# jasperlinthorst/reveal

Measured on AMD Instinct MI355X. Metric: Mbp/s indexed+MUM-anchored (reveal rem), higher is better.
Workload: dtype int32

## Files before the change

### reveal_amd/csrc/rv_cascade.hip

```cpp
#include "rv_index.h"
#include "rv_cascade.h"
#include "rv_leaf.h"
#include <algorithm>
#include <string.h>
#include <stdio.h>
#include <stdlib.h>
#include <chrono>

namespace {

constexpr int TB = 256;
constexpr u32 NONE = 0xFFFFFFFFu;
#ifdef RV_SA64
constexpr int KEY_SHIFT = 40;
#else
constexpr int KEY_SHIFT = 32;
#endif
constexpr u64 KEY_LOW = (1ull << KEY_SHIFT) - 1;

struct CasIv { sa_t a0, a1, b0, b1; };
struct CasRes { sa_t qa, qb; u32 ql, lead, trail, state; };
enum { C_NCHILD = 0, C_NUND = 1, C_NWIT = 2, C_ERR = 3, C_MAXN = 4, C_LO = 5, C_HI = 6, C_LEVELS = 7, C_NSOLVED = 8, C_NUNSOLVED = 9, C_NRETRY = 10, C_TICKET = 11,
       C_NANCH = 12  };

// ... 14 lines not shown
__device__ inline u64 shfl_up64(u64 v, int d) {
    const u32 lo = __shfl_up((u32)v, d, 64), hi = __shfl_up((u32)(v >> 32), d, 64);
    return ((u64)hi << 32) | lo;
}
__device__ inline void seg_atomic_max64(u64 *__restrict__ dst, u32 child, u64 val, bool active) {
    const int lane = threadIdx.x & 63;
    if (!active) { child = NONE; val = 0; }
    val = rv_wave_seg_max_u64(child, val);
    const u32 nc = __shfl_down(child, 1, 64);
    const bool last = lane == 63 || nc != child;
    if (active && last && val > dst[child]) atomicMax((unsigned long long *)&dst[child], (unsigned long long)val);
}
__device__ inline void seg_atomic_max32(u32 *__restrict__ dst, u32 child, u32 val, bool active) {
    const int lane = threadIdx.x & 63;
    if (!active) { child = NONE; val = 0; }
    val = rv_wave_seg_max_u32(child, val);
    const u32 nc = __shfl_down(child, 1, 64);
    const bool last = lane == 63 || nc != child;
    if (active && last && val > dst[child]) atomicMax(&dst[child], val);
}

constexpr int WT_ITEMS = 8;
constexpr int WT_TILE = TB * WT_ITEMS;
constexpr int WT_REGIONS = 64;
__global__ __launch_bounds__(TB) void k_cas_witness(const sa_t *__restrict__ SA, const lcp_t *__restrict__ LCP, const uint8_t *__restrict__ BWT, int64_t n,
                                                    u32 minl, sa_t *__restrict__ w_pos, u32 *__restrict__ w_val, u32 *__restrict__ w_rank, u32 cap , u32 *__restrict__ counters ) {
    __shared__ __attribute__((aligned(16))) u32 sl0[WT_TILE + 8];
    __shared__ __attribute__((aligned(16))) uint8_t ss0[WT_TILE + 32];
    u32 *const sl = sl0 + 3;
    uint8_t *const ss = ss0 + 15;
    const int64_t j0 = (int64_t)blockIdx.x * WT_TILE;
    if (j0 + WT_TILE + 2 <= n && sizeof(lcp_t) == 4) {
        const uint4 *L4 = reinterpret_cast<const uint4 *>(LCP + j0);
        uint4 *d4 = reinterpret_cast<uint4 *>(sl + 1);
        for (int k = threadIdx.x; k < WT_TILE / 4; k += TB) d4[k] = L4[k];
        const uint4 *B4 = reinterpret_cast<const uint4 *>(BWT + j0);
        for (int k = threadIdx.x; k < WT_TILE / 16; k += TB) {
            uint4 v = B4[k];
            v.x = (v.x >> 7) & 0x01010101u; v.y = (v.y >> 7) & 0x01010101u; v.z = (v.z >> 7) & 0x01010101u; v.w = (v.w >> 7) & 0x01010101u;
            reinterpret_cast<uint4 *>(ss + 1)[k] = v;
        }
        if (threadIdx.x == 0) { sl[0] = j0 > 0 ? (u32)LCP[j0 - 1] : 0u; ss[0] = j0 > 0 ? (uint8_t)(BWT[j0 - 1] >> 7) : (uint8_t)0; }
        if (threadIdx.x == 1) { sl[WT_TILE + 1] = (u32)LCP[j0 + WT_TILE]; ss[WT_TILE + 1] = (uint8_t)(BWT[j0 + WT_TILE] >> 7); }
        if (threadIdx.x == 2) sl[WT_TILE + 2] = (u32)LCP[j0 + WT_TILE + 1];
    } else {
        for (int k = threadIdx.x; k < WT_TILE + 3; k += TB) { const int64_t j = j0 - 1 + k; sl[k] = (j >= 0 && j < n) ? (u32)LCP[j] : 0u; }
        for (int k = threadIdx.x; k < WT_TILE + 2; k += TB) { const int64_t j = j0 - 1 + k; ss[k] = (j >= 0 && j < n) ? (uint8_t)(BWT[j] >> 7) : (uint8_t)0; }
// ... 773 lines not shown
    std::sort(CA.begin(), CA.end(), [](const RvIntv &x, const RvIntv &y) { return x.begin < y.begin; });
    std::sort(CB.begin(), CB.end(), [](const RvIntv &x, const RvIntv &y) { return x.begin < y.begin; });
    if (CA.empty() || CB.empty()) GIVE_UP("an empty sample");
    const bool chain = CA.size() > 1 || CB.size() > 1;
    if (chain && ws.opt.no_cascade_chain) GIVE_UP("several sequences per sample (switched off)");
    if (n >= ((int64_t)1 << 32) - 2) GIVE_UP("index above 2^32 positions");
#ifdef RV_SA64
    if ((u64)h->maxlcp >= (1ull << 24) || n >= ((int64_t)1 << 40)) GIVE_UP("bid word too narrow");
#endif
    CasIv root; root.a0 = root.a1 = root.b0 = root.b1 = 0;
    root.a0 = (sa_t)CA[0].begin; root.a1 = (sa_t)CA[0].end; root.b0 = (sa_t)CB[0].begin; root.b1 = (sa_t)CB[0].end;
    if (root.a0 >= root.a1 || root.b0 >= root.b1 || (int64_t)root.a1 > h->nsep[0] || (int64_t)root.b0 <= h->nsep[0]) GIVE_UP("an empty sample");

    const sa_t *SA = h->dSA.as<sa_t>(); const lcp_t *LCP = h->dLCP.as<lcp_t>(); const uint8_t *BWT = h->dBWT.as<uint8_t>();

    const int64_t ntile = ceil_div(n, RV_PAIR_TILE);
    DBuf &bcnt = ws.misc[14], &btab = ws.misc[2], &bslot = ws.misc[3], &bovf = ws.misc[4], &bout = ws.misc[5];
    if (bcnt.cap == 0) { RV_TRY(bcnt.reserve(64)); RV_HIP(hipMemsetAsync(bcnt.p, 0, 64, q)); }
    RV_TRY(btab.reserve((size_t)(ntile + 1) * 3 * sizeof(u32)));
    RV_TRY(bslot.reserve((size_t)ntile * RV_PAIR_SLOTS * sizeof(RvPairRec)));
    if (bovf.cap < 4096 * sizeof(RvPairRec)) RV_TRY(bovf.reserve(4096 * sizeof(RvPairRec)));
    if (bout.cap < 4096 * sizeof(RvPairRec)) RV_TRY(bout.reserve(sizeof(RvPairRec) * (size_t)std::max<int64_t>(4096, n / 64)));
    u32 *tilecnt = btab.as<u32>(), *tileovf = tilecnt + (ntile + 1), *tileoff = tileovf + (ntile + 1);
    u32 M = reuse ? cb.M : 0;
    for (int attempt = 0; !reuse; attempt++) {
        if (attempt == 3) { rv_set_error("cascade: scan buffer sizing failed"); return -1; }
        const size_t ocap = bout.cap / sizeof(RvPairRec) - RV_PAIR_HDR, vcap = bovf.cap / sizeof(RvPairRec);
        hipEvent_t ev_a, ev_b;
        (void)h->prof.attach(RV_K_SCAN_PAIR, (double)n * 8.0, &ev_a, &ev_b);
        RV_TRY(rv_scan_pair_launch(ws, SA, LCP, n, BWT, (sa_t)h->nsep[0], (int)minl, bslot.as<RvPairRec>(), bovf.as<RvPairRec>(),
                                   (u32)std::min<size_t>(vcap, 0xffffffffu), bcnt.as<u32>(), tilecnt, tileovf, nullptr, nullptr, 0, ev_a, ev_b));
        RV_TRY(rv_exclusive_sum_u32(ws, tilecnt, tileoff, ntile + 1));
        RV_TRY(rv_pair_compact_launch(ws, bslot.as<RvPairRec>(), bovf.as<RvPairRec>(), tilecnt, tileovf, tileoff, ntile, bout.as<RvPairRec>(),
                                      (u32)std::min<size_t>(ocap, 0xffffffffu), bcnt.as<u32>(), nullptr, (u32)std::min<size_t>(vcap, 0xffffffffu)));
        u32 hdr[4];
        RV_TRY(rv_read_back(ws, hdr, bout.p, sizeof hdr));
        const u32 total = hdr[0], novf = hdr[1];
        if (total <= ocap && novf <= vcap) { M = total; break; }
        if (novf > vcap) RV_TRY(bovf.reserve((size_t)novf * sizeof(RvPairRec)));
        if (total > ocap) RV_TRY(bout.reserve(((size_t)total + RV_PAIR_HDR) * sizeof(RvPairRec)));
    }
    if (verbose) tp[1] = cas_now();
    out->cands = M;
    struct ProfSpan { Workspace &w; int id; ~ProfSpan() { w.prof_end(id); } } span{ws, ws.prof_begin(RV_K_CASCADE, 5.0 * (double)n)};
    if (M == 0) GIVE_UP("no match at the top level");
    const RvPairRec *recs = bout.as<RvPairRec>() + RV_PAIR_HDR;
    cb.M = M;

    const int64_t rcap64 = std::min<int64_t>(n / WT_REGIONS + WT_TILE, std::max<int64_t>(16384, n / 1024));
    const u32 wcap = (u32)std::min<int64_t>(rcap64 * WT_REGIONS, 0x7fffffff);
    const int64_t ccap64 = n / (int64_t)minl + 16;
    if (ccap64 >= 0x7fffffff) GIVE_UP("too many sub-indices possible");
    const u32 ccap = (u32)ccap64;
    DBuf &k0 = cb.d[0], &k1 = cb.d[1], &v0 = cb.d[2], &v1 = cb.d[3], &bpa = cb.d[4], &bpb = cb.d[5], &blen = cb.d[6], &bcc = cb.d[7], &bwp = cb.d[8], &bwv = cb.d[9],
         &bwc = cb.d[10], &biv = cb.d[11], &bbest = cb.d[12], &bwm = cb.d[13], &bdep = cb.d[14], &bres = cb.d[15], &bctr = cb.d[16], &bund = cb.d[17], &bsz = cb.d[18];
    RV_TRY(k0.reserve((size_t)M * 8)); RV_TRY(k1.reserve((size_t)M * 8)); RV_TRY(v0.reserve((size_t)M * 4)); RV_TRY(v1.reserve((size_t)M * 4));
    RV_TRY(bpa.reserve((size_t)M * sizeof(sa_t))); RV_TRY(bpb.reserve((size_t)M * sizeof(sa_t))); RV_TRY(blen.reserve((size_t)M * 4)); RV_TRY(bcc.reserve((size_t)M * 4));
    RV_TRY(bwp.reserve((size_t)wcap * sizeof(sa_t))); RV_TRY(bwv.reserve((size_t)wcap * 4)); RV_TRY(bwc.reserve((size_t)wcap * 4));
    RV_TRY(biv.reserve((size_t)ccap * sizeof(CasIv))); RV_TRY(bbest.reserve((size_t)ccap * 8)); RV_TRY(bwm.reserve((size_t)ccap * 4)); RV_TRY(bdep.reserve((size_t)ccap * 4));
    RV_TRY(bres.reserve((size_t)ccap * sizeof(CasRes))); RV_TRY(bctr.reserve(64)); RV_TRY(bund.reserve((size_t)ccap * 4));
    u32 *counters = bctr.as<u32>();
    RV_HIP(hipMemsetAsync(counters, 0, 64, q));

    DBuf &bwp0 = cb.d[19], &bwv0 = cb.d[20], &bwr = cb.d[21], &bwrk = cb.d[22], &bwrk0 = cb.d[23];
    RV_TRY(bwp0.reserve((size_t)wcap * sizeof(sa_t))); RV_TRY(bwv0.reserve((size_t)wcap * 4)); RV_TRY(bwr.reserve(2 * WT_REGIONS * 4 + 64));
    RV_TRY(bwrk.reserve((size_t)wcap * 4)); RV_TRY(bwrk0.reserve((size_t)wcap * 4));
    u32 hc[16];
    u32 NW = reuse ? cb.NW : 0;
    if (!reuse) {
        u32 *wreg = bwr.as<u32>();
        RV_HIP(hipMemsetAsync(wreg, 0, 2 * WT_REGIONS * 4, q));
        const u32 wrcap = wcap / WT_REGIONS;
        hipLaunchKernelGGL(k_cas_witness, dim3((unsigned)ceil_div(n, WT_TILE)), dim3(TB), 0, q, SA, LCP, BWT, n, minl, bwp0.as<sa_t>(), bwv0.as<u32>(), bwrk0.as<u32>(), wrcap, wreg);
        RV_LAUNCH_CHECK();
        {
            const unsigned mb = (unsigned)ceil_div((int64_t)M, TB);
            hipLaunchKernelGGL(k_cas_keys, dim3(mb), dim3(TB), 0, q, recs, M, k0.as<u64>(), v0.as<u32>());
            RV_LAUNCH_CHECK();
            int in1 = 0;
            RV_TRY(rv_radix_sort_pairs<u32>(ws, k0.as<u64>(), v0.as<u32>(), k1.as<u64>(), v1.as<u32>(), (int64_t)M, 0, bitlen64((u64)n), &in1));
            hipLaunchKernelGGL(k_cas_gather, dim3(mb), dim3(TB), 0, q, recs, (const u32 *)(in1 ? v1.as<u32>() : v0.as<u32>()), M, bpa.as<sa_t>(), bpb.as<sa_t>(),
                               blen.as<u32>(), bcc.as<u32>());
            RV_LAUNCH_CHECK();
        }
        u32 hreg[2 * WT_REGIONS];
        RV_TRY(rv_read_back(ws, hreg, wreg, WT_REGIONS * 4));
        u32 wmaxc = 0;
        for (int r = 0; r < WT_REGIONS; r++) { hreg[WT_REGIONS + r] = NW; NW += hreg[r]; wmaxc = std::max(wmaxc, hreg[r]); }
        out->witnesses = NW;
        if (wmaxc > wrcap) GIVE_UP("too many repeat witnesses (a repetitive input)");
        if (NW) {
            RV_HIP(hipMemcpyAsync(wreg + WT_REGIONS, hreg + WT_REGIONS, WT_REGIONS * 4, hipMemcpyHostToDevice, q));
            RV_HIP(hipStreamSynchronize(q));
            hipLaunchKernelGGL(k_cas_wpack, dim3((unsigned)std::max<int64_t>(1, ceil_div((int64_t)wmaxc, TB)), WT_REGIONS), dim3(TB), 0, q, (const sa_t *)bwp0.as<sa_t>(),
                               (const u32 *)bwv0.as<u32>(), (const u32 *)bwrk0.as<u32>(), wrcap, (const u32 *)wreg, (const u32 *)(wreg + WT_REGIONS), bwp.as<sa_t>(), bwv.as<u32>(),
                               bwrk.as<u32>());
            RV_LAUNCH_CHECK();
        }
        cb.NW = NW;
        if (chain) {
            const char *why = nullptr;
            RV_TRY(cas_lineage(h, cb, M, NW, minl, CA, CB, &why));
            if (why) { cb.lin_picks = 0; cb.lin_rest.clear(); GIVE_UP(why); }
        }
    } else {
        if (chain && cb.lin_picks == 0) GIVE_UP("the chain of rest sub-indices was not decided");
        RV_HIP(hipMemsetAsync(bcc.p, 0, (size_t)M * 4, q));
        out->witnesses = NW;
    }
    const sa_t *wp = bwp.as<sa_t>(); const u32 *wv = bwv.as<u32>();
    CasDanger dg; memset(&dg, 0, sizeof dg);
    u32 dwalk_nmed = 0; const u32 *dwalk_boff = nullptr, *dwalk_mlist = nullptr;
    if (danger) {
        if (NW) {
            RV_TRY(k0.reserve((size_t)NW * 8)); RV_TRY(k1.reserve((size_t)NW * 8)); RV_TRY(v0.reserve((size_t)NW * 4)); RV_TRY(v1.reserve((size_t)NW * 4));
            const unsigned wb = (unsigned)ceil_div((int64_t)NW, TB);
            hipLaunchKernelGGL(k_cas_wkeys, dim3(wb), dim3(TB), 0, q, (const u32 *)bwrk.as<u32>(), NW, k0.as<u64>(), v0.as<u32>());
            RV_LAUNCH_CHECK();
            int in1 = 0;
            RV_TRY(rv_radix_sort_pairs<u32>(ws, k0.as<u64>(), v0.as<u32>(), k1.as<u64>(), v1.as<u32>(), (int64_t)NW, 0, bitlen64((u64)n), &in1));
// ... 207 lines not shown
```

### reveal_amd/csrc/rv_common.h

```cpp
#pragma once
#include <mutex>
#include <thread>
#include <vector>
#include <utility>
#include <hip/hip_runtime.h>
#include <stdint.h>
#include <string.h>
#include <stddef.h>
#include <vector>
#include <string>

#ifdef RV_SA64
typedef int64_t  sa_t;
typedef uint32_t lcp_t;
#else
typedef int32_t  sa_t;
typedef int32_t  lcp_t;
#endif

typedef unsigned long long u64;
typedef unsigned int       u32;

void rv_set_error(const char *fmt, ...);

// ... 51 lines not shown
    X(no_text_jump, "RV_NO_TEXT_JUMP", 0) \
    X(far_table, "RV_FAR_TABLE", 0) \
    X(no_slow_class, "RV_NO_SLOW_CLASS", 0) \
    X(no_dwalk_blocks, "RV_NO_DWALK_BLOCKS", 0) \
    X(no_pub_twins, "RV_NO_PUB_TWINS", 0) \
    X(sa_no_text, "RV_SA_NO_TEXT", 0) \
    X(text_mode, "RV_TEXT_MODE", -1) \
    X(carry_ch, "RV_CARRY_CH", -1) \
    X(rs_bits, "RV_RS_BITS", 8) \
    X(rs_xcd, "RV_RS_XCD", 1) \
    X(rs_cnt16, "RV_RS_CNT16", 1) \
    X(rs_no_digit_bytes, "RV_RS_NO_DIGIT_BYTES", 0) \
    X(diag_table, "RV_DIAG_TABLE", -1) \
    X(no_cascade_chain, "RV_NO_CASCADE_CHAIN", 0) \
    X(casm_rank_count, "RV_CASM_RANK_COUNT", 0) \
    X(casm_big_min, "RV_CASM_BIG_MIN", -1) \
    X(casm_no_big, "RV_CASM_NO_BIG", 0) \
    X(casm_big_root, "RV_CASM_BIG_ROOT", 1 << 22) \
    X(casm_big_total, "RV_CASM_BIG_TOTAL", 1 << 26) \
    X(lock_any, "RV_LOCK_ANY", 0) \
    X(presel_dev_min, "RV_PRESEL_DEV_MIN", 65536) \
    X(scan_v1, "RV_SCAN_V1", 0) \
    X(pick_threads, "RV_PICK_THREADS", 0) \
    X(cascade_prio, "RV_CASCADE_PRIO", 0)
struct RvOptions {
#define RV_X_(f, name, def) int64_t f = def;
    RV_OPTION_LIST(RV_X_)
#undef RV_X_
    int64_t *find(const char *name) {
#define RV_X_(f, nm, def) if (strcmp(name, nm) == 0) return &f;
        RV_OPTION_LIST(RV_X_)
#undef RV_X_
        return nullptr;
    }
};
extern int g_rv_launch_trace;
static inline bool rv_launch_trace_on() { return g_rv_launch_trace != 0; }
#define RV_LAUNCH_CHECK()                                                                      \
    do {                                                                                       \
        RV_HIP(hipGetLastError());                                                             \
        if (rv_launch_trace_on()) {                                                            \
            fprintf(stderr, "launch %s:%d\n", __FILE__, __LINE__);                             \
            fflush(stderr);                                                                    \
            RV_HIP(hipDeviceSynchronize());                                                    \
        }                                                                                      \
    } while (0)

// ... 191 lines not shown
        for (auto &b : sa) b.release();
    }
};

std::mutex &rv_trim_mutex();
struct SaScratchInUse {
    Workspace &w; bool was;
    SaScratchInUse(Workspace &x) : w(x) { std::lock_guard<std::mutex> g(rv_trim_mutex()); was = w.sa_in_use; w.sa_in_use = true; }
    ~SaScratchInUse() { std::lock_guard<std::mutex> g(rv_trim_mutex()); w.sa_in_use = was; }
};

int rv_exclusive_sum_u32(Workspace &ws, const u32 *in, u32 *out, int64_t n);
int rv_exclusive_sum_u64(Workspace &ws, const u64 *in, u64 *out, int64_t n);
int rv_inclusive_max_u32(Workspace &ws, const u32 *in, u32 *out, int64_t n);
int rv_inclusive_max_u64(Workspace &ws, const u64 *in, u64 *out, int64_t n);

int rv_radix_passes(const Workspace &ws, int nbits);
template <class V>
int rv_radix_sort_pairs(Workspace &ws, u64 *k0, V *v0, u64 *k1, V *v1, int64_t n,
                        int bit_lo, int bit_hi, int *result_in_1, bool first_digits = false);
uint8_t *rv_radix_first_digits(Workspace &ws, int64_t n, int bit_lo, int bit_hi);

int rv_read_back(Workspace &ws, void *dst, const void *dsrc, size_t bytes);

int rv_h2d_copy(Workspace &ws, const void *pinned_src, void *dst, size_t bytes);

struct RvSaStats {
    int    sigma, bits, k0;
    int    rounds;
    int64_t sorted_elems;
    int    radix_passes;
    int    diag_table;
    int64_t far_pairs;
    int64_t lcp_list;
};
int rv_build_sa(Workspace &ws, const uint8_t *T, int64_t n, sa_t *SA, RvSaStats *st,
                lcp_t *LCP = nullptr, uint8_t *BWT = nullptr, sa_t side_sep = 0, u32 *d_maxlcp = nullptr, bool *fused_done = nullptr,
                const int64_t *seps = nullptr, int nseps = 0);
int rv_build_inverse(Workspace &ws, const sa_t *SA, sa_t *SAi, int64_t n);
int rv_build_inverse_checked(Workspace &ws, const sa_t *SA, sa_t *SAi, int64_t n);
int rv_build_lcp(Workspace &ws, const uint8_t *T, const sa_t *SA, bool by_rank, lcp_t *LCP, int64_t n, u32 *d_maxlcp, uint8_t *BWT, sa_t side_sep);
int rv_build_bwt(Workspace &ws, const uint8_t *T, const sa_t *SA, int64_t n, uint8_t *BWT, sa_t side_sep);
```

### reveal_amd/csrc/rv_prims.hip

```cpp
#include "rv_common.h"
#include <string.h>

namespace {

constexpr int SCAN_THREADS = 256;
constexpr int SCAN_ITEMS   = 8;
constexpr int SCAN_TILE    = SCAN_THREADS * SCAN_ITEMS;

template <class T> struct OpSum {
    __device__ static T id() { return (T)0; }
    __device__ static T f(T a, T b) { return a + b; }
};
template <class T> struct OpMax {
    __device__ static T id() { return (T)0; }
    __device__ static T f(T a, T b) { return a > b ? a : b; }
};

template <class T> __device__ inline T shfl_up_t(T v, int d) { return __shfl_up(v, d, 64); }
template <> __device__ inline u64 shfl_up_t<u64>(u64 v, int d) {
    u32 lo = __shfl_up((u32)v, d, 64), hi = __shfl_up((u32)(v >> 32), d, 64);
    return ((u64)hi << 32) | lo;
}

template <class T, class Op>
// ... 336 lines not shown
        have_digits = dn != nullptr;
        u64 *tk = ki; ki = ko; ko = tk;
        V *tv = vi; vi = vo; vo = tv;
        flip ^= 1;
    }
    *result_in_1 = flip;
    return 0;
}

__global__ __launch_bounds__(256) void k_h2d_copy(const uint4 *__restrict__ src, uint4 *__restrict__ dst, size_t n16) {
    for (size_t i = (size_t)blockIdx.x * 256 + threadIdx.x; i < n16; i += (size_t)gridDim.x * 256) dst[i] = src[i];
}
int rv_read_back(Workspace &ws, void *dst, const void *dsrc, size_t bytes) {
    RV_TRY(ws.hpin.reserve(bytes < 4096 ? 4096 : bytes));
    if (!ws.ev_rb) RV_HIP(hipEventCreateWithFlags(&ws.ev_rb, hipEventDisableTiming));
    RV_HIP(hipMemcpyAsync(ws.hpin.p, dsrc, bytes, hipMemcpyDeviceToHost, ws.stream));
    RV_HIP(hipEventRecord(ws.ev_rb, ws.stream));
    const hipError_t e = rv_event_wait(ws.ev_rb);
    if (e != hipSuccess) { rv_set_error("rv_read_back: %s", hipGetErrorString(e)); return -1; }
    memcpy(dst, ws.hpin.p, bytes);
    return 0;
}

int rv_h2d_copy(Workspace &ws, const void *pinned_src, void *dst, size_t bytes) {
    const size_t n16 = (bytes + 15) / 16;
    if (n16 == 0) return 0;
    size_t blocks = (n16 + 255) / 256;
    if (blocks > 512) blocks = 512;
    hipLaunchKernelGGL(k_h2d_copy, dim3((unsigned)blocks), dim3(256), 0, ws.stream, (const uint4 *)pinned_src, (uint4 *)dst, n16);
    RV_LAUNCH_CHECK();
    return 0;
}

template int rv_radix_sort_pairs<u32>(Workspace &, u64 *, u32 *, u64 *, u32 *, int64_t, int, int, int *, bool);
template int rv_radix_sort_pairs<u64>(Workspace &, u64 *, u64 *, u64 *, u64 *, int64_t, int, int, int *, bool);
```

### reveal_amd/csrc/rv_scan.h

```cpp
#pragma once
#include "rv_common.h"

#ifndef RV_PAIR_TILE
#define RV_PAIR_TILE 1024
#endif
#define RV_TSUB_TILE 2048

struct RvPairRec {
    sa_t a, b;
    u32  l;
    u32  rank;
};

#define RV_PAIR_SLOTS 16
int rv_scan_pair_launch(Workspace &ws, const sa_t *SA, const lcp_t *LCP, int64_t m, const uint8_t *BWT, sa_t nsep0, int minl,
                        RvPairRec *slots, RvPairRec *ovf, u32 ovf_cap, u32 *ovf_counter, u32 *tilecnt, u32 *tileovf,
                        unsigned long long *best, RvPairRec *picks, int nsubs,
                        hipEvent_t ev_start = nullptr, hipEvent_t ev_stop = nullptr);
int rv_pick_slots_launch(Workspace &ws, const RvPairRec *slots, const RvPairRec *ovf, u32 ovf_cap, const u32 *tilecnt, const u32 *tileovf, int64_t ntile,
                         const int64_t *sub_start, int nsubs, unsigned long long *best, RvPairRec *picks, u32 *ovf_counter, const u32 *err,
                         const int *tile_sub, int64_t ntsub);
#define RV_PAIR_HDR 1
int rv_pair_compact_launch(Workspace &ws, const RvPairRec *slots, const RvPairRec *ovf, const u32 *tilecnt, const u32 *tileovf,
                           const u32 *tileoff, int64_t ntile, RvPairRec *out, u32 out_cap, u32 *ovf_counter, const u32 *err, u32 ovf_cap);

#define RV_MULTI_TILE 512
struct RvMultiRec { u32 l, n, ub, pad; };
int rv_scan_multi_launch(Workspace &ws, const sa_t *SA, const lcp_t *LCP, int64_t m, const uint8_t *BWT, const sa_t *nsep, int nsamples,
                         int minl, int minn, RvMultiRec *rec, uint16_t *so, sa_t *pos, u32 rec_cap, u32 mem_cap, u32 *counters, uint4 *tiletab,
                         const int64_t *sub_start, const int *sub_want, int nsubs);

#define RV_MEMS_MAX_SAMPLES 65536
int rv_multimems_launch(Workspace &ws, const sa_t *SA, const lcp_t *LCP, const uint8_t *BWT, int64_t n, const sa_t *nsep, int nsamples, int minl, int minn,
                        u32 maxlcp, u32 *rec_l, int32_t *rec_c, int64_t *rec_first, uint16_t *so, sa_t *pos,
                        unsigned long long rec_cap, unsigned long long mem_cap, unsigned long long *out);

struct RvMultiCand;
int rv_multi_pick_launch(Workspace &ws, const sa_t *SA, const lcp_t *LCP, int64_t m, const uint8_t *BWT, const sa_t *nsep, int nsamples, int minl, int minn,
                         const int64_t *sub_start, const int *sub_want, int nsubs, const int *tile_sub ,
                         unsigned long long *best, u32 *pick_l, sa_t *pick_pos, RvMultiCand *cand, u32 cand_cap, u32 *cand_count,
                         hipEvent_t ev_start = nullptr, hipEvent_t ev_stop = nullptr);
// ... 5 lines not shown
```

### reveal_amd/csrc/rv_scan.hip

```cpp
#include "rv_common.h"
#include "rv_scan.h"
#include <hip/hip_ext.h>
#include <algorithm>

namespace {

constexpr int TB = 256;
constexpr int PAIR_ITEMS = RV_PAIR_TILE / 64;
constexpr int PAIR_TILE = TB * PAIR_ITEMS;
__device__ inline int64_t ceil_div_dev(int64_t a, int64_t b) { return (a + b - 1) / b; }
typedef int v4i __attribute__((ext_vector_type(4)));
typedef unsigned int v2u __attribute__((ext_vector_type(2)));
typedef unsigned int v4u32 __attribute__((ext_vector_type(4)));

__device__ inline bool is_lower_c(uint8_t c) { return c >= 'a' && c <= 'z'; }

__device__ inline bool left_maximal(uint8_t ca, uint8_t cb) {
    return (ca != cb) || ca == 'N' || ca == '$' || is_lower_c(ca);
}

__device__ inline bool lcp_lt(lcp_t v, int minl) {
#ifdef RV_SA64
    return v < (lcp_t)minl;
#else
// ... 17 lines not shown
    __builtin_amdgcn_fence(__ATOMIC_ACQUIRE, "wavefront");
#pragma unroll
    for (int j = 0; j < 4; j++) {
        const uint4 t = corner[lane * LT_ROW + j];
        out[4 * j] = t.x; out[4 * j + 1] = t.y; out[4 * j + 2] = t.z; out[4 * j + 3] = t.w;
    }
}

__device__ inline u32 pair_bytes4(u32 x, u32 y) {
    const u32 K = 0x7f7f7f7fu;
    const u32 xc = x & K, yc = y & K;
    const u32 ne = (xc ^ yc) + K;
    const u32 plain = ((xc ^ 0x4e4e4e4eu) + K) & ((xc ^ 0x24242424u) + K);
    const u32 low = (xc + 0x1f1f1f1fu) & ~(xc + 0x05050505u);
    return (x ^ y) & (ne | ~plain | low) & 0x80808080u;
}
__device__ inline u32 bits4_of_bytes(u32 e) {
    u32 v = (e >> 7) & 0x01010101u;
    v |= v >> 7;
    v |= v >> 14;
    return v & 0xfu;
}

__global__ __launch_bounds__(TB) void k_scan_pair(const sa_t *__restrict__ SA, const lcp_t *__restrict__ LCP, int64_t m,
                                                  const uint8_t *__restrict__ BWT, sa_t nsep0, int minl,
                                                  RvPairRec *__restrict__ slots, RvPairRec *__restrict__ ovf, u32 ovf_cap,
                                                  u32 *__restrict__ ovf_counter, u32 *__restrict__ tilecnt, u32 *__restrict__ tileovf,
                                                  unsigned long long *__restrict__ best, RvPairRec *__restrict__ picks, int nsubs) {
    static_assert(PAIR_ITEMS == 16, "sixteen ranks per lane: four 16-byte loads of LCP, one of BWT");
    const int lane = threadIdx.x & 63, w = threadIdx.x >> 6;
    const int64_t tile = blockIdx.x;
    const int64_t i0 = tile * PAIR_TILE + (int64_t)threadIdx.x * PAIR_ITEMS;
    if (blockIdx.x == 0 && threadIdx.x == 0) tilecnt[ceil_div_dev(m, RV_PAIR_TILE)] = 0;
    for (int64_t s2 = (int64_t)blockIdx.x * TB + threadIdx.x; s2 < nsubs; s2 += (int64_t)gridDim.x * TB) { best[s2] = 0; picks[RV_PAIR_HDR + s2].rank = 0xFFFFFFFFu; }

    const int64_t wfirst = __builtin_amdgcn_readfirstlane((int)(threadIdx.x & ~63)) * (int64_t)PAIR_ITEMS + tile * PAIR_TILE;
    const int64_t wnext = wfirst + 64 * PAIR_ITEMS;
    u32 h_lc = 0, h_nlc = 0, h_bw = 0;
    if (wfirst > 0 && wfirst - 1 < m) { h_lc = (u32)LCP[wfirst - 1]; h_bw = BWT[wfirst - 1]; }
    if (wnext < m) h_nlc = (u32)LCP[wnext];

    __shared__ uint4 s_corner[TB / 64][64 * LT_ROW];
    u32 lc[PAIR_ITEMS + 2], bx[PAIR_ITEMS / 4];
    if (wnext <= m) {
        const v4u32 bb = __builtin_nontemporal_load(reinterpret_cast<const v4u32 *>(BWT + i0));
        bx[0] = bb.x; bx[1] = bb.y; bx[2] = bb.z; bx[3] = bb.w;
        wave_lcp16(LCP, wfirst, lane, s_corner[w], lc + 1);
    } else {
#pragma unroll
        for (int k = 0; k < PAIR_ITEMS / 4; k++) bx[k] = 0;
#pragma unroll
        for (int k = 0; k < PAIR_ITEMS; k++) {
            lc[1 + k] = (i0 + k < m) ? (u32)LCP[i0 + k] : 0u;
            bx[k >> 2] |= ((i0 + k < m) ? (u32)BWT[i0 + k] : 0u) << (8 * (k & 3));
        }
    }
    lc[0] = (u32)__shfl_up((int)lc[PAIR_ITEMS], 1, 64);
    lc[PAIR_ITEMS + 1] = (u32)__shfl_down((int)lc[1], 1, 64);
    u32 plast = (u32)__shfl_up((int)bx[PAIR_ITEMS / 4 - 1], 1, 64);
    if (lane == 0) { lc[0] = h_lc; plast = h_bw << 24; }
    if (lane == 63) lc[PAIR_ITEMS + 1] = h_nlc;

#ifdef RV_SA64
    const u32 thr = minl < 0 ? 0xFFFFFFFFu : (minl >= 1 ? (u32)minl - 1u : 0u);
#else
    const u32 thr = minl >= 1 ? (u32)minl - 1u : 0u;
#endif
    u32 hit = 0;
#pragma unroll
    for (int k = 0; k < PAIR_ITEMS; k++) {
        const u32 a = lc[k], c = lc[k + 2];
        u32 mx = a > c ? a : c;
        mx = mx > thr ? mx : thr;
        hit |= (u32)(lc[k + 1] > mx) << k;
    }
    u32 okb = 0;
#pragma unroll
    for (int k = 0; k < PAIR_ITEMS / 4; k++) {
        const u32 y = __builtin_amdgcn_alignbit(bx[k], k ? bx[k - 1] : plast, 24);
        okb |= bits4_of_bytes(pair_bytes4(bx[k], y)) << (4 * k);
    }
    hit &= okb;
    const u32 mine = __popc(hit);
    const u32 inc = rv_wave_incl_sum_u32(mine);
    const u32 tot = (u32)__builtin_amdgcn_readlane((int)inc, 63);
    const int64_t wtile = tile * (TB / 64) + w;
    if (wfirst >= m) return;
    u32 base = 0;
    if (lane == 0) {
        if (tot > RV_PAIR_SLOTS) base = atomicAdd(ovf_counter, tot - RV_PAIR_SLOTS);
        tilecnt[wtile] = tot;
        tileovf[wtile] = base;
    }
    base = (u32)__shfl((int)base, 0, 64);
    u32 hh = hit, q = inc - mine;
    while (hh) {
        const int k = __builtin_ctz(hh);
        hh &= hh - 1;
        const sa_t s1 = SA[i0 + k], s0 = SA[i0 + k - 1];
        RvPairRec r;
        r.a = s1 < s0 ? s1 : s0;
        r.b = s1 < s0 ? s0 : s1;
        r.l = (u32)LCP[i0 + k];
        r.rank = (u32)(i0 + k);
        if (q < RV_PAIR_SLOTS) slots[(size_t)wtile * RV_PAIR_SLOTS + q] = r;
        else { const u32 o = base + (q - RV_PAIR_SLOTS); if (o < ovf_cap) ovf[o] = r; }
        q++;
    }
}

__global__ __launch_bounds__(TB) void k_pair_compact(const RvPairRec *__restrict__ slots, const RvPairRec *__restrict__ ovf,
                                                     const u32 *__restrict__ tilecnt, const u32 *__restrict__ tileovf,
                                                     const u32 *__restrict__ tileoff, int64_t ntile, RvPairRec *__restrict__ out, u32 out_cap,
                                                     u32 *__restrict__ ovf_counter, const u32 *__restrict__ err, u32 ovf_cap) {
    const int64_t id = (int64_t)blockIdx.x * TB + threadIdx.x;
    if (id == 0) {
        u32 *hdr = reinterpret_cast<u32 *>(out);
        hdr[0] = tileoff[ntile]; hdr[1] = *ovf_counter; hdr[2] = err ? *err : 0u; hdr[3] = 0;
        *ovf_counter = 0;
    }
    out += RV_PAIR_HDR;
    const int64_t t = id / RV_PAIR_SLOTS;
    const u32 j = (u32)(id % RV_PAIR_SLOTS);
    if (t >= ntile) return;
    const u32 cnt = tilecnt[t];
    if (j >= cnt) return;
    const u32 o = tileoff[t];
    if (o + j < out_cap) out[o + j] = slots[(size_t)t * RV_PAIR_SLOTS + j];
    const u32 ob = tileovf[t];
    for (u32 q = RV_PAIR_SLOTS + j; q < cnt; q += RV_PAIR_SLOTS)
// ... 657 lines not shown
                              sub_start, sub_want, nsubs, tile_sub, best, pick_l, cand, cand_cap, cand_count);
    else
        hipLaunchKernelGGL(k_multi_pick1, dim3((unsigned)ceil_div(m, RV_TSUB_TILE)), dim3(TB), 0, ws.stream, SA, LCP, m, BWT, nsep, nsamples, minl, minn,
                           sub_start, sub_want, nsubs, tile_sub, best, pick_l, cand, cand_cap, cand_count);
    RV_LAUNCH_CHECK();
    hipLaunchKernelGGL(k_multi_pick2, dim3(RV_MULTI_REGIONS * 4), dim3(TB), 0, ws.stream, SA, sub_want, nsamples, (const unsigned long long *)best,
                       (const RvMultiCand *)cand, cand_cap, (const u32 *)cand_count, pick_l, pick_pos);
    RV_LAUNCH_CHECK();
    return 0;
}

int rv_scan_multi_launch(Workspace &ws, const sa_t *SA, const lcp_t *LCP, int64_t m, const uint8_t *BWT, const sa_t *nsep, int nsamples,
                         int minl, int minn, RvMultiRec *rec, uint16_t *so, sa_t *pos, u32 rec_cap, u32 mem_cap, u32 *counters, uint4 *tiletab,
                         const int64_t *sub_start, const int *sub_want, int nsubs) {
    if (m <= 0) return 0;
    hipLaunchKernelGGL(k_scan_multi, dim3((unsigned)ceil_div(m, (int64_t)RV_MULTI_TILE * (TB / 64))), dim3(TB), 0, ws.stream, SA, LCP, m, BWT, nsep, nsamples, minl, minn,
                       rec, so, pos, rec_cap, mem_cap, counters, tiletab, sub_start, sub_want, nsubs);
    RV_LAUNCH_CHECK();
    return 0;
}

int rv_scan_pair_launch(Workspace &ws, const sa_t *SA, const lcp_t *LCP, int64_t m, const uint8_t *BWT, sa_t nsep0, int minl,
                        RvPairRec *slots, RvPairRec *ovf, u32 ovf_cap, u32 *ovf_counter, u32 *tilecnt, u32 *tileovf,
                        unsigned long long *best, RvPairRec *picks, int nsubs, hipEvent_t ev_start, hipEvent_t ev_stop) {
    if (m <= 0) return 0;
    const int64_t nb = ceil_div(m, PAIR_TILE);
    if (ev_start && ev_stop)
        hipExtLaunchKernelGGL(k_scan_pair, dim3((unsigned)nb), dim3(TB), 0, ws.stream, ev_start, ev_stop, 0, SA, LCP, m, BWT, nsep0, minl, slots, ovf, ovf_cap, ovf_counter,
                              tilecnt, tileovf, best, picks, nsubs);
    else
        hipLaunchKernelGGL(k_scan_pair, dim3((unsigned)nb), dim3(TB), 0, ws.stream, SA, LCP, m, BWT, nsep0, minl, slots, ovf, ovf_cap, ovf_counter, tilecnt, tileovf,
                           best, picks, nsubs);
    RV_LAUNCH_CHECK();
    return 0;
}

int rv_pick_slots_launch(Workspace &ws, const RvPairRec *slots, const RvPairRec *ovf, u32 ovf_cap, const u32 *tilecnt, const u32 *tileovf, int64_t ntile,
                          const int64_t *sub_start, int nsubs, unsigned long long *best, RvPairRec *picks, u32 *ovf_counter, const u32 *err,
                          const int *tile_sub, int64_t ntsub) {
    if (ntile <= 0 || nsubs <= 0) return 0;
    const unsigned g = (unsigned)ceil_div(ntile * RV_PAIR_SLOTS, TB);
    hipLaunchKernelGGL(k_pick_slots<1>, dim3(g), dim3(TB), 0, ws.stream, slots, ovf, ovf_cap, tilecnt, tileovf, ntile, sub_start, nsubs, best, picks, ovf_counter, err, tile_sub, ntsub);
    RV_LAUNCH_CHECK();
    hipLaunchKernelGGL(k_pick_slots<2>, dim3(g), dim3(TB), 0, ws.stream, slots, ovf, ovf_cap, tilecnt, tileovf, ntile, sub_start, nsubs, best, picks, ovf_counter, err, tile_sub, ntsub);
    RV_LAUNCH_CHECK();
    return 0;
}

int rv_pair_compact_launch(Workspace &ws, const RvPairRec *slots, const RvPairRec *ovf, const u32 *tilecnt, const u32 *tileovf,
                           const u32 *tileoff, int64_t ntile, RvPairRec *out, u32 out_cap, u32 *ovf_counter, const u32 *err, u32 ovf_cap) {
    if (ntile <= 0) return 0;
    hipLaunchKernelGGL(k_pair_compact, dim3((unsigned)ceil_div(ntile * RV_PAIR_SLOTS, TB)), dim3(TB), 0, ws.stream, slots, ovf, tilecnt, tileovf,
                       tileoff, ntile, out, out_cap, ovf_counter, err, ovf_cap);
    RV_LAUNCH_CHECK();
    return 0;
// ... 2 lines not shown
```

Baseline: 23130.

## Fuse repeat-witness detection into the pair scan kernel

Computes witness bitmasks inside k_scan_pair (templated on WIT) and writes witness records into per-region buffers during the same pass over SA/LCP/BWT, so the separate k_cas_witness pass over the whole index is skipped by default. The region counts are read back together with the scan header in one combined readback, which removes a host round trip. In exchange the scan kernel takes on extra bit logic, more registers and scattered LCP/SA loads for each witness. The old separate pass stays available behind RV_CAS_WITNESS_PASS.

```diff
diff --git a/reveal_amd/csrc/rv_cascade.hip b/reveal_amd/csrc/rv_cascade.hip
--- a/reveal_amd/csrc/rv_cascade.hip
+++ b/reveal_amd/csrc/rv_cascade.hip
@@ -60,7 +60,7 @@
 
 constexpr int WT_ITEMS = 8;
 constexpr int WT_TILE = TB * WT_ITEMS;
-constexpr int WT_REGIONS = 64;
+constexpr int WT_REGIONS = RV_WIT_REGIONS;
 __global__ __launch_bounds__(TB) void k_cas_witness(const sa_t *__restrict__ SA, const lcp_t *__restrict__ LCP, const uint8_t *__restrict__ BWT, int64_t n,
                                                     u32 minl, sa_t *__restrict__ w_pos, u32 *__restrict__ w_val, u32 *__restrict__ w_rank, u32 cap , u32 *__restrict__ counters ) {
     __shared__ __attribute__((aligned(16))) u32 sl0[WT_TILE + 8];
@@ -880,19 +880,31 @@
     if (bovf.cap < 4096 * sizeof(RvPairRec)) RV_TRY(bovf.reserve(4096 * sizeof(RvPairRec)));
     if (bout.cap < 4096 * sizeof(RvPairRec)) RV_TRY(bout.reserve(sizeof(RvPairRec) * (size_t)std::max<int64_t>(4096, n / 64)));
     u32 *tilecnt = btab.as<u32>(), *tileovf = tilecnt + (ntile + 1), *tileoff = tileovf + (ntile + 1);
+    const bool wit_pass = ws.opt.cas_witness_pass != 0;
+    const int64_t wtile = wit_pass ? WT_TILE : RV_PAIR_WG_TILE;
+    const int64_t rcap64 = std::min<int64_t>(n / WT_REGIONS + wtile, std::max<int64_t>(16384, n / 1024));
+    const u32 wcap = (u32)std::min<int64_t>(rcap64 * WT_REGIONS, 0x7fffffff);
+    const u32 wrcap = wcap / WT_REGIONS;
+    DBuf &bwp0 = cb.d[19], &bwv0 = cb.d[20], &bwr = cb.d[21], &bwrk = cb.d[22], &bwrk0 = cb.d[23];
+    u32 hreg[2 * WT_REGIONS];
+    RV_TRY(bwp0.reserve((size_t)wcap * sizeof(sa_t))); RV_TRY(bwv0.reserve((size_t)wcap * 4)); RV_TRY(bwr.reserve(2 * WT_REGIONS * 4 + 64));
+    RV_TRY(bwrk.reserve((size_t)wcap * 4)); RV_TRY(bwrk0.reserve((size_t)wcap * 4));
+    const RvScanWit swit = {bwp0.as<sa_t>(), bwv0.as<u32>(), bwrk0.as<u32>(), wrcap, bwr.as<u32>()};
     u32 M = reuse ? cb.M : 0;
     for (int attempt = 0; !reuse; attempt++) {
         if (attempt == 3) { rv_set_error("cascade: scan buffer sizing failed"); return -1; }
         const size_t ocap = bout.cap / sizeof(RvPairRec) - RV_PAIR_HDR, vcap = bovf.cap / sizeof(RvPairRec);
+        if (!wit_pass) RV_HIP(hipMemsetAsync(bwr.p, 0, 2 * WT_REGIONS * 4, q));
         hipEvent_t ev_a, ev_b;
         (void)h->prof.attach(RV_K_SCAN_PAIR, (double)n * 8.0, &ev_a, &ev_b);
         RV_TRY(rv_scan_pair_launch(ws, SA, LCP, n, BWT, (sa_t)h->nsep[0], (int)minl, bslot.as<RvPairRec>(), bovf.as<RvPairRec>(),
-                                   (u32)std::min<size_t>(vcap, 0xffffffffu), bcnt.as<u32>(), tilecnt, tileovf, nullptr, nullptr, 0, ev_a, ev_b));
+                                   (u32)std::min<size_t>(vcap, 0xffffffffu), bcnt.as<u32>(), tilecnt, tileovf, nullptr, nullptr, 0, ev_a, ev_b, wit_pass ? nullptr : &swit));
         RV_TRY(rv_exclusive_sum_u32(ws, tilecnt, tileoff, ntile + 1));
         RV_TRY(rv_pair_compact_launch(ws, bslot.as<RvPairRec>(), bovf.as<RvPairRec>(), tilecnt, tileovf, tileoff, ntile, bout.as<RvPairRec>(),
                                       (u32)std::min<size_t>(ocap, 0xffffffffu), bcnt.as<u32>(), nullptr, (u32)std::min<size_t>(vcap, 0xffffffffu)));
         u32 hdr[4];
-        RV_TRY(rv_read_back(ws, hdr, bout.p, sizeof hdr));
+        if (wit_pass) RV_TRY(rv_read_back(ws, hdr, bout.p, sizeof hdr));
+        else RV_TRY(rv_read_back2(ws, hdr, bout.p, sizeof hdr, hreg, bwr.p, WT_REGIONS * 4));
         const u32 total = hdr[0], novf = hdr[1];
         if (total <= ocap && novf <= vcap) { M = total; break; }
         if (novf > vcap) RV_TRY(bovf.reserve((size_t)novf * sizeof(RvPairRec)));
@@ -900,13 +912,11 @@
     }
     if (verbose) tp[1] = cas_now();
     out->cands = M;
-    struct ProfSpan { Workspace &w; int id; ~ProfSpan() { w.prof_end(id); } } span{ws, ws.prof_begin(RV_K_CASCADE, 5.0 * (double)n)};
+    struct ProfSpan { Workspace &w; int id; ~ProfSpan() { w.prof_end(id); } } span{ws, ws.prof_begin(RV_K_CASCADE, (wit_pass ? 5.0 * (double)n : 0.0) + 16.0 * (double)M)};
     if (M == 0) GIVE_UP("no match at the top level");
     const RvPairRec *recs = bout.as<RvPairRec>() + RV_PAIR_HDR;
     cb.M = M;
 
-    const int64_t rcap64 = std::min<int64_t>(n / WT_REGIONS + WT_TILE, std::max<int64_t>(16384, n / 1024));
-    const u32 wcap = (u32)std::min<int64_t>(rcap64 * WT_REGIONS, 0x7fffffff);
     const int64_t ccap64 = n / (int64_t)minl + 16;
     if (ccap64 >= 0x7fffffff) GIVE_UP("too many sub-indices possible");
     const u32 ccap = (u32)ccap64;
@@ -920,17 +930,31 @@
     u32 *counters = bctr.as<u32>();
     RV_HIP(hipMemsetAsync(counters, 0, 64, q));
 
-    DBuf &bwp0 = cb.d[19], &bwv0 = cb.d[20], &bwr = cb.d[21], &bwrk = cb.d[22], &bwrk0 = cb.d[23];
-    RV_TRY(bwp0.reserve((size_t)wcap * sizeof(sa_t))); RV_TRY(bwv0.reserve((size_t)wcap * 4)); RV_TRY(bwr.reserve(2 * WT_REGIONS * 4 + 64));
-    RV_TRY(bwrk.reserve((size_t)wcap * 4)); RV_TRY(bwrk0.reserve((size_t)wcap * 4));
     u32 hc[16];
     u32 NW = reuse ? cb.NW : 0;
     if (!reuse) {
         u32 *wreg = bwr.as<u32>();
-        RV_HIP(hipMemsetAsync(wreg, 0, 2 * WT_REGIONS * 4, q));
-        const u32 wrcap = wcap / WT_REGIONS;
-        hipLaunchKernelGGL(k_cas_witness, dim3((unsigned)ceil_div(n, WT_TILE)), dim3(TB), 0, q, SA, LCP, BWT, n, minl, bwp0.as<sa_t>(), bwv0.as<u32>(), bwrk0.as<u32>(), wrcap, wreg);
-        RV_LAUNCH_CHECK();
+        u32 wmaxc = 0;
+        auto pack = [&]() -> int {
+            for (int r = 0; r < WT_REGIONS; r++) { hreg[WT_REGIONS + r] = NW; NW += hreg[r]; wmaxc = std::max(wmaxc, hreg[r]); }
+            out->witnesses = NW;
+            if (wmaxc > wrcap || NW == 0) return 0;
+            RV_HIP(hipMemcpyAsync(wreg + WT_REGIONS, hreg + WT_REGIONS, WT_REGIONS * 4, hipMemcpyHostToDevice, q));
+            RV_HIP(hipStreamSynchronize(q));
+            hipLaunchKernelGGL(k_cas_wpack, dim3((unsigned)std::max<int64_t>(1, ceil_div((int64_t)wmaxc, TB)), WT_REGIONS), dim3(TB), 0, q, (const sa_t *)bwp0.as<sa_t>(),
+                               (const u32 *)bwv0.as<u32>(), (const u32 *)bwrk0.as<u32>(), wrcap, (const u32 *)wreg, (const u32 *)(wreg + WT_REGIONS), bwp.as<sa_t>(), bwv.as<u32>(),
+                               bwrk.as<u32>());
+            RV_LAUNCH_CHECK();
+            return 0;
+        };
+        if (wit_pass) {
+            RV_HIP(hipMemsetAsync(wreg, 0, 2 * WT_REGIONS * 4, q));
+            hipLaunchKernelGGL(k_cas_witness, dim3((unsigned)ceil_div(n, WT_TILE)), dim3(TB), 0, q, SA, LCP, BWT, n, minl, bwp0.as<sa_t>(), bwv0.as<u32>(), bwrk0.as<u32>(), wrcap, wreg);
+            RV_LAUNCH_CHECK();
+        } else {
+            RV_TRY(pack());
+            if (wmaxc > wrcap) GIVE_UP("too many repeat witnesses (a repetitive input)");
+        }
         {
             const unsigned mb = (unsigned)ceil_div((int64_t)M, TB);
             hipLaunchKernelGGL(k_cas_keys, dim3(mb), dim3(TB), 0, q, recs, M, k0.as<u64>(), v0.as<u32>());
@@ -941,19 +965,10 @@
                                blen.as<u32>(), bcc.as<u32>());
             RV_LAUNCH_CHECK();
         }
-        u32 hreg[2 * WT_REGIONS];
-        RV_TRY(rv_read_back(ws, hreg, wreg, WT_REGIONS * 4));
-        u32 wmaxc = 0;
-        for (int r = 0; r < WT_REGIONS; r++) { hreg[WT_REGIONS + r] = NW; NW += hreg[r]; wmaxc = std::max(wmaxc, hreg[r]); }
-        out->witnesses = NW;
-        if (wmaxc > wrcap) GIVE_UP("too many repeat witnesses (a repetitive input)");
-        if (NW) {
-            RV_HIP(hipMemcpyAsync(wreg + WT_REGIONS, hreg + WT_REGIONS, WT_REGIONS * 4, hipMemcpyHostToDevice, q));
-            RV_HIP(hipStreamSynchronize(q));
-            hipLaunchKernelGGL(k_cas_wpack, dim3((unsigned)std::max<int64_t>(1, ceil_div((int64_t)wmaxc, TB)), WT_REGIONS), dim3(TB), 0, q, (const sa_t *)bwp0.as<sa_t>(),
-                               (const u32 *)bwv0.as<u32>(), (const u32 *)bwrk0.as<u32>(), wrcap, (const u32 *)wreg, (const u32 *)(wreg + WT_REGIONS), bwp.as<sa_t>(), bwv.as<u32>(),
-                               bwrk.as<u32>());
-            RV_LAUNCH_CHECK();
+        if (wit_pass) {
+            RV_TRY(rv_read_back(ws, hreg, wreg, WT_REGIONS * 4));
+            RV_TRY(pack());
+            if (wmaxc > wrcap) GIVE_UP("too many repeat witnesses (a repetitive input)");
         }
         cb.NW = NW;
         if (chain) {
diff --git a/reveal_amd/csrc/rv_common.h b/reveal_amd/csrc/rv_common.h
--- a/reveal_amd/csrc/rv_common.h
+++ b/reveal_amd/csrc/rv_common.h
@@ -97,7 +97,8 @@
     X(presel_dev_min, "RV_PRESEL_DEV_MIN", 65536) \
     X(scan_v1, "RV_SCAN_V1", 0) \
     X(pick_threads, "RV_PICK_THREADS", 0) \
-    X(cascade_prio, "RV_CASCADE_PRIO", 0)
+    X(cascade_prio, "RV_CASCADE_PRIO", 0) \
+    X(cas_witness_pass, "RV_CAS_WITNESS_PASS", 0)
 struct RvOptions {
 #define RV_X_(f, name, def) int64_t f = def;
     RV_OPTION_LIST(RV_X_)
@@ -335,6 +336,7 @@
 uint8_t *rv_radix_first_digits(Workspace &ws, int64_t n, int bit_lo, int bit_hi);
 
 int rv_read_back(Workspace &ws, void *dst, const void *dsrc, size_t bytes);
+int rv_read_back2(Workspace &ws, void *dst_a, const void *dsrc_a, size_t bytes_a, void *dst_b, const void *dsrc_b, size_t bytes_b);
 
 int rv_h2d_copy(Workspace &ws, const void *pinned_src, void *dst, size_t bytes);
 
diff --git a/reveal_amd/csrc/rv_prims.hip b/reveal_amd/csrc/rv_prims.hip
--- a/reveal_amd/csrc/rv_prims.hip
+++ b/reveal_amd/csrc/rv_prims.hip
@@ -382,6 +382,20 @@
     return 0;
 }
 
+int rv_read_back2(Workspace &ws, void *dst_a, const void *dsrc_a, size_t bytes_a, void *dst_b, const void *dsrc_b, size_t bytes_b) {
+    const size_t off = (bytes_a + 63) & ~(size_t)63;
+    RV_TRY(ws.hpin.reserve(off + bytes_b < 4096 ? 4096 : off + bytes_b));
+    if (!ws.ev_rb) RV_HIP(hipEventCreateWithFlags(&ws.ev_rb, hipEventDisableTiming));
+    RV_HIP(hipMemcpyAsync(ws.hpin.p, dsrc_a, bytes_a, hipMemcpyDeviceToHost, ws.stream));
+    RV_HIP(hipMemcpyAsync((uint8_t *)ws.hpin.p + off, dsrc_b, bytes_b, hipMemcpyDeviceToHost, ws.stream));
+    RV_HIP(hipEventRecord(ws.ev_rb, ws.stream));
+    const hipError_t e = rv_event_wait(ws.ev_rb);
+    if (e != hipSuccess) { rv_set_error("rv_read_back2: %s", hipGetErrorString(e)); return -1; }
+    memcpy(dst_a, ws.hpin.p, bytes_a);
+    memcpy(dst_b, (const uint8_t *)ws.hpin.p + off, bytes_b);
+    return 0;
+}
+
 int rv_h2d_copy(Workspace &ws, const void *pinned_src, void *dst, size_t bytes) {
     const size_t n16 = (bytes + 15) / 16;
     if (n16 == 0) return 0;
diff --git a/reveal_amd/csrc/rv_scan.h b/reveal_amd/csrc/rv_scan.h
--- a/reveal_amd/csrc/rv_scan.h
+++ b/reveal_amd/csrc/rv_scan.h
@@ -13,10 +13,14 @@
 };
 
 #define RV_PAIR_SLOTS 16
+#define RV_WIT_REGIONS 64
+#define RV_PAIR_WG_TILE (4 * RV_PAIR_TILE)
+struct RvScanWit { sa_t *pos; u32 *val; u32 *rank; u32 cap; u32 *counters; };
 int rv_scan_pair_launch(Workspace &ws, const sa_t *SA, const lcp_t *LCP, int64_t m, const uint8_t *BWT, sa_t nsep0, int minl,
                         RvPairRec *slots, RvPairRec *ovf, u32 ovf_cap, u32 *ovf_counter, u32 *tilecnt, u32 *tileovf,
                         unsigned long long *best, RvPairRec *picks, int nsubs,
-                        hipEvent_t ev_start = nullptr, hipEvent_t ev_stop = nullptr);
+                        hipEvent_t ev_start = nullptr, hipEvent_t ev_stop = nullptr,
+                        const RvScanWit *wit = nullptr);
 int rv_pick_slots_launch(Workspace &ws, const RvPairRec *slots, const RvPairRec *ovf, u32 ovf_cap, const u32 *tilecnt, const u32 *tileovf, int64_t ntile,
                          const int64_t *sub_start, int nsubs, unsigned long long *best, RvPairRec *picks, u32 *ovf_counter, const u32 *err,
                          const int *tile_sub, int64_t ntsub);
diff --git a/reveal_amd/csrc/rv_scan.hip b/reveal_amd/csrc/rv_scan.hip
--- a/reveal_amd/csrc/rv_scan.hip
+++ b/reveal_amd/csrc/rv_scan.hip
@@ -63,11 +63,12 @@
     return v & 0xfu;
 }
 
+template <bool WIT>
 __global__ __launch_bounds__(TB) void k_scan_pair(const sa_t *__restrict__ SA, const lcp_t *__restrict__ LCP, int64_t m,
                                                   const uint8_t *__restrict__ BWT, sa_t nsep0, int minl,
                                                   RvPairRec *__restrict__ slots, RvPairRec *__restrict__ ovf, u32 ovf_cap,
                                                   u32 *__restrict__ ovf_counter, u32 *__restrict__ tilecnt, u32 *__restrict__ tileovf,
-                                                  unsigned long long *__restrict__ best, RvPairRec *__restrict__ picks, int nsubs) {
+                                                  unsigned long long *__restrict__ best, RvPairRec *__restrict__ picks, int nsubs, RvScanWit wit) {
     static_assert(PAIR_ITEMS == 16, "sixteen ranks per lane: four 16-byte loads of LCP, one of BWT");
     const int lane = threadIdx.x & 63, w = threadIdx.x >> 6;
     const int64_t tile = blockIdx.x;
@@ -80,6 +81,11 @@
     u32 h_lc = 0, h_nlc = 0, h_bw = 0;
     if (wfirst > 0 && wfirst - 1 < m) { h_lc = (u32)LCP[wfirst - 1]; h_bw = BWT[wfirst - 1]; }
     if (wnext < m) h_nlc = (u32)LCP[wnext];
+    u32 h_nlc2 = 0, h_nbw = 0;
+    if constexpr (WIT) {
+        if (wnext < m) h_nbw = BWT[wnext];
+        if (wnext + 1 < m) h_nlc2 = (u32)LCP[wnext + 1];
+    }
 
     __shared__ uint4 s_corner[TB / 64][64 * LT_ROW];
     u32 lc[PAIR_ITEMS + 2], bx[PAIR_ITEMS / 4];
@@ -120,6 +126,33 @@
     for (int k = 0; k < PAIR_ITEMS / 4; k++) {
         const u32 y = __builtin_amdgcn_alignbit(bx[k], k ? bx[k - 1] : plast, 24);
         okb |= bits4_of_bytes(pair_bytes4(bx[k], y)) << (4 * k);
+    }
+    u32 wit16 = 0, wp0 = 0, wp1 = 0;
+    if constexpr (WIT) {
+        u32 g = 0, d = 0;
+#pragma unroll
+        for (int k = 0; k < PAIR_ITEMS; k++) g |= (u32)(lc[k + 1] > thr) << k;
+#pragma unroll
+        for (int k = 0; k < PAIR_ITEMS / 4; k++) {
+            const u32 y = __builtin_amdgcn_alignbit(bx[k], k ? bx[k - 1] : plast, 24);
+            d |= bits4_of_bytes(bx[k] ^ y) << (4 * k);
+        }
+        u32 u = hit & d;
+        if (i0 == 0) u &= ~1u;
+        const u32 pack = g | (u << 16);
+        u32 prev = (u32)__shfl_up((int)pack, 1, 64), next = (u32)__shfl_down((int)pack, 1, 64);
+        if (lane == 0) prev = (u32)(h_lc > thr) << 15;
+        if (lane == 63) {
+            u32 mx = lc[PAIR_ITEMS] > h_nlc2 ? lc[PAIR_ITEMS] : h_nlc2;
+            mx = mx > thr ? mx : thr;
+            const u32 un = (u32)(h_nlc > mx) & (((h_nbw << 24) ^ bx[PAIR_ITEMS / 4 - 1]) >> 31);
+            next = (u32)(h_nlc > thr) | ((u32)(h_nlc2 > thr) << 1) | (un << 16);
+        }
+        const u32 gw = ((prev >> 15) & 1u) | (g << 1) | ((next & 3u) << 17);
+        wp0 = u;
+        wp1 = ((u >> 1) | ((next >> 16) << 15)) & ~wp0;
+        wit16 = ((wp0 & (gw | (gw >> 2))) | (wp1 & ((gw >> 1) | (gw >> 3))) | (~(wp0 | wp1) & ((gw >> 1) | (gw >> 2)))) & 0xffffu;
+        if (i0 + PAIR_ITEMS > m) wit16 &= i0 < m ? (1u << (int)(m - i0)) - 1u : 0u;
     }
     hit &= okb;
     const u32 mine = __popc(hit);
@@ -147,6 +180,26 @@
         if (q < RV_PAIR_SLOTS) slots[(size_t)wtile * RV_PAIR_SLOTS + q] = r;
         else { const u32 o = base + (q - RV_PAIR_SLOTS); if (o < ovf_cap) ovf[o] = r; }
         q++;
+    }
+    if constexpr (WIT) {
+        if (__ballot(wit16 != 0)) {
+            const u32 cnt = __popc(wit16);
+            const u32 winc = rv_wave_incl_sum_u32(cnt);
+            const u32 reg = blockIdx.x & (RV_WIT_REGIONS - 1);
+            u32 wbase = 0;
+            if (lane == 63) wbase = atomicAdd(&wit.counters[reg], winc);
+            u32 o = (u32)__shfl((int)wbase, 63, 64) + winc - cnt;
+            u32 ww = wit16;
+            while (ww) {
+                const int k = __builtin_ctz(ww);
+                ww &= ww - 1;
+                const int64_t j = i0 + k;
+                const u32 lm1 = j >= 1 ? (u32)LCP[j - 1] : 0u, l0 = (u32)LCP[j], l1 = j + 1 < m ? (u32)LCP[j + 1] : 0u, l2 = j + 2 < m ? (u32)LCP[j + 2] : 0u;
+                const u32 v = ((wp0 >> k) & 1u) ? (lm1 > l1 ? lm1 : l1) : ((wp1 >> k) & 1u) ? (l0 > l2 ? l0 : l2) : (l0 > l1 ? l0 : l1);
+                if (o < wit.cap) { const size_t f = (size_t)reg * wit.cap + o; wit.pos[f] = SA[j]; wit.val[f] = v; wit.rank[f] = (u32)j; }
+                o++;
+            }
+        }
     }
 }
 
@@ -850,15 +903,18 @@
 
 int rv_scan_pair_launch(Workspace &ws, const sa_t *SA, const lcp_t *LCP, int64_t m, const uint8_t *BWT, sa_t nsep0, int minl,
                         RvPairRec *slots, RvPairRec *ovf, u32 ovf_cap, u32 *ovf_counter, u32 *tilecnt, u32 *tileovf,
-                        unsigned long long *best, RvPairRec *picks, int nsubs, hipEvent_t ev_start, hipEvent_t ev_stop) {
+                        unsigned long long *best, RvPairRec *picks, int nsubs, hipEvent_t ev_start, hipEvent_t ev_stop, const RvScanWit *wit) {
     if (m <= 0) return 0;
+    static_assert(PAIR_TILE == RV_PAIR_WG_TILE, "rv_scan.h names the workgroup's stretch of ranks");
     const int64_t nb = ceil_div(m, PAIR_TILE);
+    const auto kern = wit ? k_scan_pair<true> : k_scan_pair<false>;
+    const RvScanWit w = wit ? *wit : RvScanWit{nullptr, nullptr, nullptr, 0, nullptr};
     if (ev_start && ev_stop)
-        hipExtLaunchKernelGGL(k_scan_pair, dim3((unsigned)nb), dim3(TB), 0, ws.stream, ev_start, ev_stop, 0, SA, LCP, m, BWT, nsep0, minl, slots, ovf, ovf_cap, ovf_counter,
-                              tilecnt, tileovf, best, picks, nsubs);
+        hipExtLaunchKernelGGL(kern, dim3((unsigned)nb), dim3(TB), 0, ws.stream, ev_start, ev_stop, 0, SA, LCP, m, BWT, nsep0, minl, slots, ovf, ovf_cap, ovf_counter,
+                              tilecnt, tileovf, best, picks, nsubs, w);
     else
-        hipLaunchKernelGGL(k_scan_pair, dim3((unsigned)nb), dim3(TB), 0, ws.stream, SA, LCP, m, BWT, nsep0, minl, slots, ovf, ovf_cap, ovf_counter, tilecnt, tileovf,
-                           best, picks, nsubs);
+        hipLaunchKernelGGL(kern, dim3((unsigned)nb), dim3(TB), 0, ws.stream, SA, LCP, m, BWT, nsep0, minl, slots, ovf, ovf_cap, ovf_counter, tilecnt, tileovf,
+                           best, picks, nsubs, w);
     RV_LAUNCH_CHECK();
     return 0;
 }
```

New measurement: 23760 (median of 6 runs). 2.7% higher.
